# kdexd/virtex

Hardware: NVIDIA H100
Metric: image-caption pairs/sec bicaptioning R50-L1-H1024 (higher is better)
Workload: dtype bf16

## Files before the change

virtex_b200/csrc/gemm_tc.cu:

```cuda
#include <stdlib.h>
#include "ptx.cuh"
#include "vtx_common.cuh"
#include "../../include/virtex_b200.h"

#define KP_TAPS_W p.taps_w
#define KP_PAD p.pad
#define KP_NTAPS p.ntaps

namespace vtx {

constexpr int kBM = 128;
constexpr int kBK = 64;
constexpr int kMaxStages = 8;
constexpr int kABytes = kBM * kBK * 2;
constexpr int kSmemTotal = 232448;
constexpr int kCtrlBytes = 1024;
constexpr int kThreads = 384;
constexpr int kEpiThreads = 256;

struct FastDiv {
  uint32_t mul, shr;
};
__device__ __forceinline__ int fdiv(int x, const FastDiv& f) {
  return f.mul == 0u ? x : (int)(__umulhi((uint32_t)x, f.mul) >> f.shr);
// ... 675 lines not shown
        const int slabs = (min(p.bn, p.N - n_base) + 63) >> 6;
        for (int sl = 0; sl < slabs; ++sl) {
          if (p.mode & 1)
            tma_store_4d(&tmD, cbuf + sl * 16384, n_base + sl * 64, tw << p.lbw, th << p.lbh, tn << p.lbn);
          else
            tma_store_2d(&tmD, cbuf + sl * 16384, n_base + sl * 64, mt * kBM);
        }
        tma_store_commit();
      }
      if (bnr_on) {
        const uint32_t cp = smem_u32(cbuf) + (scg >> 3) * 16384 + bnr_r0 * 128;
        const int c8 = scg & 7;
        float mean[8], sc[8], sh[8];
        {
          const float4 m0 = __ldg(reinterpret_cast<const float4*>(p.bnr_bnp + bnr_col));
          const float4 m1 = __ldg(reinterpret_cast<const float4*>(p.bnr_bnp + bnr_col + 4));
          mean[0] = m0.x; mean[1] = m0.y; mean[2] = m0.z; mean[3] = m0.w;
          mean[4] = m1.x; mean[5] = m1.y; mean[6] = m1.z; mean[7] = m1.w;
          const float4 a0 = __ldg(reinterpret_cast<const float4*>(p.bnr_bnp + 2 * p.N + bnr_col));
          const float4 a1 = __ldg(reinterpret_cast<const float4*>(p.bnr_bnp + 2 * p.N + bnr_col + 4));
          const float4 b0 = __ldg(reinterpret_cast<const float4*>(p.bnr_bnp + 3 * p.N + bnr_col));
          const float4 b1 = __ldg(reinterpret_cast<const float4*>(p.bnr_bnp + 3 * p.N + bnr_col + 4));
          sc[0] = a0.x; sc[1] = a0.y; sc[2] = a0.z; sc[3] = a0.w; sc[4] = a1.x; sc[5] = a1.y; sc[6] = a1.z; sc[7] = a1.w;
          sh[0] = b0.x; sh[1] = b0.y; sh[2] = b0.z; sh[3] = b0.w; sh[4] = b1.x; sh[5] = b1.y; sh[6] = b1.z; sh[7] = b1.w;
        }
        for (int rb = 0; rb < st_rpt; rb += 4) {
          uint4 yv[4];
          uint32_t mbits;
          bnr_load(rb, yv, mbits);
#pragma unroll
          for (int r4 = 0; r4 < 4; ++r4) {
            const int r = rb + r4;
            const uint4 raw = lds128(cp + r * 128 + ((c8 ^ ((bnr_r0 + r) & 7)) << 4));
            float f[8], yy[8];
            unpack8(*reinterpret_cast<const bf16x8*>(&raw), f);
            unpack8(*reinterpret_cast<const bf16x8*>(&yv[r4]), yy);
#pragma unroll
            for (int i = 0; i < 8; ++i) {
              const bool on = p.bnr == 1 ? ((yy[i] * sc[i] + sh[i] > 0.f) && ((mbits >> (8 * r4)) & 0xffu) != 0u)
                                         : (((mbits >> (8 * r4 + i)) & 1u) != 0u);
              const float dz = on ? f[i] : 0.f;
              st_s[i] += dz;
              st_q[i] += dz * (yy[i] - mean[i]);
            }
          }
        }
      }
      if (!p.bnr && p.stats != nullptr && st_on) {
        const int r0 = srg * st_rpt;
        const uint32_t cp = smem_u32(cbuf) + (scg >> 3) * 16384 + r0 * 128;
        const int c8 = scg & 7;
        for (int rb = 0; rb < st_rpt; rb += 4) {
#pragma unroll
          for (int r4 = 0; r4 < 4; ++r4) {
            const int r = rb + r4;
            const uint4 raw = lds128(cp + r * 128 + ((c8 ^ ((r0 + r) & 7)) << 4));
            float f[8];
            unpack8(*reinterpret_cast<const bf16x8*>(&raw), f);
#pragma unroll
            for (int i = 0; i < 8; ++i) {
              st_s[i] += f[i];
              st_q[i] += f[i] * f[i];
            }
          }
        }
      }
    }
  }
  if (staged) {
    if (et == 0) tma_store_wait_read<0>();
    epi_bar(bar_id, epi_threads);
    if (p.stats != nullptr && st_nt >= 0) flush_stats(cstage0 + (PP ? (size_t)wg * p.cbytes : 0));
  }
}

typedef CUresult (*PFN_encodeTiled)(CUtensorMap*, CUtensorMapDataType, cuuint32_t, void*, const cuuint64_t*,
                                    const cuuint64_t*, const cuuint32_t*, const cuuint32_t*, CUtensorMapInterleave,
                                    CUtensorMapSwizzle, CUtensorMapL2promotion, CUtensorMapFloatOOBfill);

static PFN_encodeTiled get_encode() {
  static PFN_encodeTiled fn = nullptr;
  if (fn == nullptr) {
    void* p = nullptr;
    cudaDriverEntryPointQueryResult q;
    if (cudaGetDriverEntryPoint("cuTensorMapEncodeTiled", &p, cudaEnableDefault, &q) == cudaSuccess &&
        q == cudaDriverEntryPointSuccess)
      fn = reinterpret_cast<PFN_encodeTiled>(p);
  }
  return fn;
}

static int make_tmap(CUtensorMap* tm, const void* ptr, int rank, const uint64_t* dims, const uint64_t* strides_elems,
                     const uint32_t* box, const uint32_t* estr = nullptr) {
  PFN_encodeTiled enc = get_encode();
  if (!enc) return set_error(VTX_ECUDA, "cuTensorMapEncodeTiled entry point not available");
  cuuint64_t gdim[5];
  cuuint64_t gstr[5];
  cuuint32_t bx[5];
  cuuint32_t es[5];
  for (int i = 0; i < rank; ++i) {
    gdim[i] = dims[i];
    bx[i] = box[i];
    es[i] = estr ? estr[i] : 1;
  }
  for (int i = 0; i < rank - 1; ++i) gstr[i] = strides_elems[i] * 2;
  if ((reinterpret_cast<uintptr_t>(ptr) & 15) != 0) return set_error(VTX_EINVAL, "TMA base pointer not 16B aligned");
  for (int i = 0; i < rank - 1; ++i)
    if (gstr[i] % 16 != 0) return set_error(VTX_EINVAL, "TMA stride not a multiple of 16 bytes");
  CUresult r = enc(tm, CU_TENSOR_MAP_DATA_TYPE_BFLOAT16, (cuuint32_t)rank, const_cast<void*>(ptr), gdim, gstr, bx, es,
                   CU_TENSOR_MAP_INTERLEAVE_NONE, CU_TENSOR_MAP_SWIZZLE_128B, CU_TENSOR_MAP_L2_PROMOTION_L2_256B,
                   CU_TENSOR_MAP_FLOAT_OOB_FILL_NONE);
  if (r != CUDA_SUCCESS) return set_error(VTX_ECUDA, "cuTensorMapEncodeTiled failed (%d)", (int)r);
  return VTX_OK;
}

constexpr int kSchedSlots = 4096;
static int g_sched_dynamic = 0;
static struct SchedRing {
  unsigned int* ctr;
  unsigned int base[kSchedSlots];
  unsigned int next;
} g_sched[64];
static bool sched_is_dynamic() {
  static const char* env = getenv("VTX_GEMM_SCHEDULE");
  return env != nullptr ? (env[0] == 'd') : (g_sched_dynamic != 0);
}
static unsigned int* sched_slot(unsigned int fetches, unsigned int* base_out) {
  if (!sched_is_dynamic()) return nullptr;
  int dev = 0;
  cudaGetDevice(&dev);
  if (dev < 0 || dev >= 64) return nullptr;
  SchedRing& r = g_sched[dev];
  if (r.ctr == nullptr) {
    unsigned int* ptr = nullptr;
    if (cudaMalloc(&ptr, sizeof(unsigned int) * kSchedSlots) != cudaSuccess) return nullptr;
    cudaMemset(ptr, 0, sizeof(unsigned int) * kSchedSlots);
    cudaDeviceSynchronize();
    memset(r.base, 0, sizeof(r.base));
    r.next = 0;
    r.ctr = ptr;
  }
  const unsigned int slot = r.next++ % kSchedSlots;
  *base_out = r.base[slot];
  r.base[slot] += fetches;
  return r.ctr + slot;
}

static int ilog2(int x) {
  int l = 0;
  while ((1 << l) < x) ++l;
  return l;
}

static void choose_box(int H, int W, int positions, int* bw, int* bh, int* bn) {
  int best_w = 1, best_h = 1;
  double best_eff = -1;
  for (int w = 1; w <= positions; w <<= 1)
    for (int h = 1; w * h <= positions; h <<= 1) {
      if (w > 2 * W || h > 2 * H) continue;
      const int tw = (W + w - 1) / w, th = (H + h - 1) / h;
      const double eff = (double)(W * H) / ((double)tw * w * th * h);
      const double score = eff * 1000.0 + w * 0.01 + h * 0.0001;
      if (score > best_eff) { best_eff = score; best_w = w; best_h = h; }
    }
  *bw = best_w; *bh = best_h; *bn = positions / (best_w * best_h);
}

template <bool SS>
static cudaError_t launch_gemm(const cudaLaunchConfig_t& cfg, bool pingpong, int bn, const CUtensorMap& tmA,
                               const CUtensorMap& tmB, const CUtensorMap& tmD, const CUtensorMap& tmR,
                               const CUtensorMap& tmY, const GemmKParams& p) {
  if (pingpong && bn == 64) return cudaLaunchKernelEx(&cfg, gemm_wgmma_kernel<64, true, SS>, tmA, tmB, tmD, tmR, tmY, p);
  if (pingpong) return cudaLaunchKernelEx(&cfg, gemm_wgmma_kernel<128, true, SS>, tmA, tmB, tmD, tmR, tmY, p);
  if (bn == 64) return cudaLaunchKernelEx(&cfg, gemm_wgmma_kernel<64, false, SS>, tmA, tmB, tmD, tmR, tmY, p);
  if (bn == 128) return cudaLaunchKernelEx(&cfg, gemm_wgmma_kernel<128, false, SS>, tmA, tmB, tmD, tmR, tmY, p);
  if (bn == 192) return cudaLaunchKernelEx(&cfg, gemm_wgmma_kernel<192, false, SS>, tmA, tmB, tmD, tmR, tmY, p);
  return cudaLaunchKernelEx(&cfg, gemm_wgmma_kernel<256, false, SS>, tmA, tmB, tmD, tmR, tmY, p);
}

bool resid_dgrad_serves(const VtxGemm* g);
int resid_dgrad(const VtxGemm* g, cudaStream_t stream);

}

using namespace vtx;

extern "C" int vtx_gemm_set_dynamic_schedule(int on) {
  g_sched_dynamic = on ? 1 : 0;
  return VTX_OK;
}

extern "C" int vtx_gemm(const VtxGemm* g, void* stream_) {
  cudaStream_t stream = reinterpret_cast<cudaStream_t>(stream_);
  if (!g || !g->A || !g->B || !g->D) return set_error(VTX_EINVAL, "vtx_gemm: null pointer");
  if (g->M <= 0 || g->N <= 0 || g->K <= 0) return set_error(VTX_EINVAL, "vtx_gemm: empty problem");
  if (g->atomic && !g->out_f32) return set_error(VTX_EINVAL, "vtx_gemm: atomic accumulate needs fp32 output");
  if (g->split_k > 1 && !g->atomic) return set_error(VTX_EINVAL, "vtx_gemm: split_k > 1 needs atomic = 1");
  if (g->stats && (g->out_f32 || g->bias || g->residual || g->act || (g->alpha != 0.f && g->alpha != 1.f)))
    return set_error(VTX_EINVAL, "vtx_gemm: stats needs a plain bf16 output (no bias/residual/activation/alpha)");
  if (g->ldd % (g->out_f32 ? 4 : 8) != 0) return set_error(VTX_EINVAL, "vtx_gemm: ldd must keep rows 16B aligned");
  if (g->conv_mode < 0 || g->conv_mode > 6 || g->conv_mode == 3)
    return set_error(VTX_EINVAL, "vtx_gemm: conv_mode must be 0, 1, 2, 4, 5 or 6");
  VtxGemm g4;
  const bool trans_d = g->conv_mode == 4;
  if (trans_d) {
    if (g->conv_c != 64 || g->N != 64 || g->M != 9 * 64 || !g->out_f32 || !g->atomic)
      return set_error(VTX_EINVAL, "vtx_gemm: conv_mode 4 needs C = Cout = 64, M = 576, fp32 atomic output");
    g4 = *g;
    g4.conv_mode = 2;
    g4.M = g->N;
    g4.N = g->M;
    g4.split_k = vtx_num_sms() / 3;
    g4.conv_stride = 1;
    g4.conv_taps = 0;
    g = &g4;
  }
  const int split_k = g->split_k > 1 ? g->split_k : 1;

  GemmKParams p;
  memset(&p, 0, sizeof(p));
  p.M = g->M; p.N = g->N; p.K = g->K;
  p.a_mn = g->a_mn; p.b_mn = g->b_mn;
  p.mode = g->conv_mode;
  const bool stem = g->conv_mode == 5 || g->conv_mode == 6;
  p.taps_w = 3; p.pad = 1; p.ntaps = 9;
  if (stem) { p.mode = g->conv_mode == 5 ? 1 : 2; p.taps_w = 1; p.pad = 0; p.ntaps = 4; }
  const bool one_tap = !stem && g->conv_taps == 1;
  if (one_tap) { p.taps_w = 1; p.pad = 0; p.ntaps = 1; }
  const bool tap_grid = !stem && !one_tap && g->conv_taps_h > 0;
  if (tap_grid) {
    if (p.mode != 1 || g->conv_taps_w <= 0 || g->conv_taps_h > 3 || g->conv_taps_w > 3 || g->conv_pad < 0 || g->conv_pad > 1)
      return set_error(VTX_EINVAL, "vtx_gemm: bad explicit tap grid");
    p.taps_w = g->conv_taps_w; p.pad = g->conv_pad; p.ntaps = g->conv_taps_h * g->conv_taps_w;
  }
  const int cstride = (g->conv_stride == 2 && (p.mode == 1 || p.mode == 2) && !stem) ? 2 : 1;
  if (g->conv_stride != 0 && g->conv_stride != 1 && cstride != 2)
    return set_error(VTX_EINVAL, "vtx_gemm: conv_stride 2 is supported for conv_mode 1 / 2 only");
  if (g->conv_taps != 0 && g->conv_taps != 1 && g->conv_taps != 9) return set_error(VTX_EINVAL, "vtx_gemm: conv_taps must be 0, 1 or 9");
  p.cstride = cstride;
  const int ntaps = stem ? 4 : one_tap ? 1 : tap_grid ? p.ntaps : 9;
  if (p.mode == 1) { p.a_mn = 0; p.b_mn = 0; }
  if (p.mode == 2) { p.a_mn = 1; p.b_mn = 1; }
  int bn = g->tile_n;
  if (bn == 0) {
    const int gran = p.b_mn ? 64 : 16;
    if (g->N >= 256) bn = 256;
    else bn = ((g->N + gran - 1) / gran) * gran;
    if (bn == 256 && split_k == 1) {
      const long mt = (g->M + kBM - 1) / kBM;
      const long t256 = mt * ((g->N + 255) / 256);
      const int sms = vtx_num_sms();
      if (t256 < 100 || (t256 < sms && g->N % 256 != 0 && g->N <= 2048)) {
        bn = 128;
      } else if (t256 < 3L * sms && p.mode <= 1) {
        long best_cost = 0;
        int best_bn = 256;
        for (int cand = 256; cand >= 128; cand -= 64) {
          const long tiles = mt * ((g->N + cand - 1) / cand);
          const long cost = ((tiles + sms - 1) / sms) * (cand + 64);
          if (best_cost == 0 || cost < best_cost) { best_cost = cost; best_bn = cand; }
        }
        bn = best_bn;
      }
    }
  }
  if (bn < 16 || bn > 256 || bn % 16 != 0 || (p.b_mn && bn % 64 != 0))
    return set_error(VTX_EINVAL, "vtx_gemm: bad tile_n %d", bn);
  bn = bn <= 64 ? 64 : bn <= 128 ? 128 : bn <= 192 ? 192 : 256;
  const bool pingpong = bn <= 128 && !g->out_f32;
  p.bn = bn;
  p.n_tiles = (g->N + bn - 1) / bn;
  p.trans_d = trans_d ? 1 : 0;
  p.out_f32 = g->out_f32; p.atomic = g->atomic; p.act = g->act;
  p.alpha = g->alpha == 0.f ? 1.0f : g->alpha;
  p.D = g->D; p.ldd = g->ldd;
  p.bias = g->bias;
  p.bias_pairs = (g->bias != nullptr && g->N % 2 == 0 && (reinterpret_cast<uintptr_t>(g->bias) & 7) == 0) ? 1 : 0;
  p.residual = reinterpret_cast<const __nv_bfloat16*>(g->residual);
  p.ldr = g->ldr;
  p.res_mask = reinterpret_cast<const uint8_t*>(g->residual_mask);
  if (p.res_mask != nullptr && (g->residual == nullptr || g->N % 32 != 0 || g->conv_mode != 0 || g->out_f32 ||
                                (reinterpret_cast<uintptr_t>(g->residual_mask) & 3) != 0))
    return set_error(VTX_EINVAL, "vtx_gemm: residual_mask needs a residual, a plain bf16 GEMM and N %% 32 == 0");
  p.stats = g->stats;
  const bool bnr = g->bnr_y != nullptr;
  if (bnr) {
    if (!g->bnr_bnp || !g->bnr_sums || g->stats || g->out_f32 || g->bias || g->act || (g->alpha != 0.f && g->alpha != 1.f) ||
        g->N % 8 != 0 || g->bnr_ldy % 8 != 0 || (reinterpret_cast<uintptr_t>(g->bnr_y) & 15) != 0 ||
        (reinterpret_cast<uintptr_t>(g->bnr_bnp) & 15) != 0 || (g->bnr_mask != nullptr && g->conv_mode != 0) ||
        g->conv_mode == 2 || g->conv_mode >= 4 || split_k > 1)
      return set_error(VTX_EINVAL, "vtx_gemm: bnr needs a plain bf16 output (no stats/bias/activation/alpha/split-K), "
                                   "N %% 8 == 0, 16-byte aligned y / bnp; the bit-mask form needs conv_mode 0");
    if ((long long)g->M * (g->bnr_ldy > g->N ? g->bnr_ldy : g->N) >= (1ll << 31))
      return set_error(VTX_EUNSUPPORTED, "vtx_gemm: bnr needs M * ld(y) < 2^31");
    p.stats = g->bnr_sums;
    p.bnr_y = reinterpret_cast<const __nv_bfloat16*>(g->bnr_y);
    p.bnr_bnp = g->bnr_bnp;
    p.bnr_mask = g->bnr_mask;
    p.bnr_ldy = g->bnr_ldy;
    const char* pf = getenv("VTX_BNR_PREFETCH");
    p.bnr_prefetch = (pf != nullptr && pf[0] == '0') ? 0 : 1;
    p.bnr = g->bnr_mask == nullptr ? 1 : 2;
  }
  if (g->tile_n == 0 && resid_dgrad_serves(g)) return resid_dgrad(g, stream);
  const bool ss = g->col_scale != nullptr || g->col_shift != nullptr;
  if (ss) {
    if (!g->col_scale || !g->col_shift || g->out_f32 || (g->alpha != 0.f && g->alpha != 1.f) || g->bias || g->stats ||
        bnr || g->act < 0 || g->act > 1 || g->N % 2 != 0 || (reinterpret_cast<uintptr_t>(g->col_scale) & 7) != 0 ||
        (reinterpret_cast<uintptr_t>(g->col_shift) & 7) != 0 || g->residual_mask || g->conv_out_w > 0 ||
        (g->conv_mode != 0 && g->conv_mode != 1) ||
        (g->residual && (g->ldr % 8 != 0 || (reinterpret_cast<uintptr_t>(g->residual) & 15) != 0)))
      return set_error(VTX_EINVAL, "vtx_gemm: col_scale / col_shift need both vectors 8-byte aligned, a bf16 output, "
                                   "alpha 1, act 0 or 1, N %% 2 == 0, conv_mode 0 or 1 without an output view, no bias / "
                                   "stats / bnr / residual mask, and a 16-byte aligned residual with ldr %% 8 == 0");
    p.col_scale = g->col_scale;
    p.col_shift = g->col_shift;
  }

  CUtensorMap tmA, tmB;
  int rc;
  if (p.mode == 0) {
    p.m_tiles = (g->M + kBM - 1) / kBM;
    p.kb_total = (g->K + kBK - 1) / kBK;
    {
      uint64_t dims[2], str[1];
      uint32_t box[2];
      if (!p.a_mn) { dims[0] = g->K; dims[1] = g->M; box[0] = 64; box[1] = 128; }
      else { dims[0] = g->M; dims[1] = g->K; box[0] = 64; box[1] = 64; }
      str[0] = g->lda;
      if ((rc = make_tmap(&tmA, g->A, 2, dims, str, box)) != VTX_OK) return rc;
    }
    {
      uint64_t dims[2], str[1];
      uint32_t box[2];
      if (!p.b_mn) { dims[0] = g->K; dims[1] = g->N; box[0] = 64; box[1] = (uint32_t)bn; }
      else { dims[0] = g->N; dims[1] = g->K; box[0] = 64; box[1] = 64; }
      str[0] = g->ldb;
      if ((rc = make_tmap(&tmB, g->B, 2, dims, str, box)) != VTX_OK) return rc;
    }
  } else {
    const int C = g->conv_c, Hin = g->conv_h, Win = g->conv_w, NI = g->conv_n;
    const int H = (Hin - 1) / cstride + 1, W = (Win - 1) / cstride + 1;
    if (C <= 0 || C % 64 != 0) return set_error(VTX_EINVAL, "vtx_gemm: implicit conv needs channels %% 64 == 0");
    p.cH = H; p.cW = W; p.cN = NI; p.cpb = C / 64;
    const uint64_t xdims[4] = {(uint64_t)C, (uint64_t)Win, (uint64_t)(stem ? Hin + 3 : Hin), (uint64_t)NI};
    const uint64_t xstr[3] = {(uint64_t)(stem ? 16 : C), stem ? (uint64_t)(Win + 3) * 16 : (uint64_t)Win * C,
                              stem ? (uint64_t)(Hin + 3) * (Win + 3) * 16 : (uint64_t)Hin * Win * C};
    int bw, bh, bnn;
    choose_box(H, W, p.mode == 1 ? 128 : 64, &bw, &bh, &bnn);
    p.lbw = ilog2(bw); p.lbh = ilog2(bh); p.lbn = ilog2(bnn);
    p.tiles_w = (W + bw - 1) / bw;
    p.tiles_h = (H + bh - 1) / bh;
    const int tiles_n = (NI + bnn - 1) / bnn;
    if (p.mode == 1) {
      if (g->M != NI * H * W || g->K != ntaps * C) return set_error(VTX_EINVAL, "vtx_gemm: conv fprop shape mismatch");
      if (stem && g->stats && (W % bw != 0 || H % bh != 0))
        return set_error(VTX_EUNSUPPORTED, "vtx_gemm: conv_mode 5 with stats needs an output size tiled exactly by %dx%d", bw, bh);
      p.m_tiles = p.tiles_w * p.tiles_h * tiles_n;
      p.kb_total = ntaps * p.cpb;
      uint32_t box[4] = {64, (uint32_t)(bw * cstride), (uint32_t)(bh * cstride), (uint32_t)bnn};
      const uint32_t es[4] = {1, (uint32_t)cstride, (uint32_t)cstride, 1};
      if ((rc = make_tmap(&tmA, g->A, 4, xdims, xstr, box, cstride > 1 ? es : nullptr)) != VTX_OK) return rc;
      uint64_t bd[2] = {(uint64_t)g->K, (uint64_t)g->N};
      uint64_t bs[1] = {(uint64_t)g->ldb};
      uint32_t bb[2] = {64, (uint32_t)bn};
      if ((rc = make_tmap(&tmB, g->B, 2, bd, bs, bb)) != VTX_OK) return rc;
    } else {
      if (g->N != ntaps * C) return set_error(VTX_EINVAL, "vtx_gemm: conv wgrad shape mismatch");
      const int Cout = g->M;
      if (Cout % 64 != 0) return set_error(VTX_EINVAL, "vtx_gemm: conv wgrad needs Cout %% 64 == 0");
      p.m_tiles = (Cout + kBM - 1) / kBM;
      p.kb_total = p.tiles_w * p.tiles_h * tiles_n;
      uint64_t ad[4] = {(uint64_t)Cout, (uint64_t)W, (uint64_t)H, (uint64_t)NI};
      uint64_t as[3] = {(uint64_t)Cout, (uint64_t)W * Cout, (uint64_t)H * W * Cout};
      uint32_t box[4] = {64, (uint32_t)bw, (uint32_t)bh, (uint32_t)bnn};
      if ((rc = make_tmap(&tmA, g->A, 4, ad, as, box)) != VTX_OK) return rc;
      uint32_t xbox[4] = {64, (uint32_t)(bw * cstride), (uint32_t)(bh * cstride), (uint32_t)bnn};
      const uint32_t es[4] = {1, (uint32_t)cstride, (uint32_t)cstride, 1};
      if ((rc = make_tmap(&tmB, g->B, 4, xdims, xstr, xbox, cstride > 1 ? es : nullptr)) != VTX_OK) return rc;
    }
  }
  p.k_splits = split_k;
  if (p.k_splits > p.kb_total) p.k_splits = p.kb_total;
  p.kb_per_split = (p.kb_total + p.k_splits - 1) / p.k_splits;
  p.k_splits = (p.kb_total + p.kb_per_split - 1) / p.kb_per_split;

  p.stage_bytes = kABytes + bn * kBK * 2;
  p.cbytes = p.out_f32 ? 0 : ((bn + 63) / 64) * 16384;
  {
    const int kb_tile = p.kb_per_split;
    const int budget = kSmemTotal - 1024  - kCtrlBytes;
    int st = 0;
    p.nbuf = 1;
    if (pingpong) {
      p.nbuf = 2;
    } else if (p.cbytes) {
      const int st2 = (budget - 2 * p.cbytes) / p.stage_bytes;
      if (st2 >= 4 || (st2 >= 2 && st2 >= kb_tile)) { p.nbuf = 2; st = st2; }
    }
    if (st == 0) st = (budget - p.nbuf * p.cbytes) / p.stage_bytes;
    if (st > kMaxStages) st = kMaxStages;
    if (st < 2) return set_error(VTX_EUNSUPPORTED, "vtx_gemm: not enough shared memory for a 2-stage pipeline");
    p.stages = st;
  }
  CUtensorMap tmD, tmR, tmY;
  memset(&tmY, 0, sizeof(tmY));
  memset(&tmD, 0, sizeof(tmD));
  memset(&tmR, 0, sizeof(tmR));
  p.res_tma = (p.cbytes && g->residual != nullptr && g->ldr % 8 == 0 &&
               (reinterpret_cast<uintptr_t>(g->residual) & 15) == 0 && p.alpha == 1.0f && g->bias == nullptr &&
               (g->act == 0 || ss)) ? 1 : 0;
  if (p.cbytes) {
    if (p.mode & 1) {
      uint64_t dd[4] = {(uint64_t)g->N, (uint64_t)p.cW, (uint64_t)p.cH, (uint64_t)g->conv_n};
      uint64_t ds[3] = {(uint64_t)g->ldd, (uint64_t)p.cW * g->ldd, (uint64_t)p.cH * p.cW * g->ldd};
      if (g->conv_out_w > 0) {
        if (g->conv_out_h <= 0 || g->ldd_w % 8 || g->ldd_h % 8 || g->ldd_n % 8 || (g->residual != nullptr && !p.res_tma))
          return set_error(VTX_EINVAL, "vtx_gemm: bad output view");
        dd[1] = (uint64_t)g->conv_out_w; dd[2] = (uint64_t)g->conv_out_h;
        ds[0] = (uint64_t)g->ldd_w; ds[1] = (uint64_t)g->ldd_h; ds[2] = (uint64_t)g->ldd_n;
      }
      uint32_t db[4] = {64, 1u << p.lbw, 1u << p.lbh, 1u << p.lbn};
      if ((rc = make_tmap(&tmD, g->D, 4, dd, ds, db)) != VTX_OK) return rc;
      p.vW = (int)dd[1]; p.vH = (int)dd[2];
      if (bnr) {
        uint64_t ys[3] = {(uint64_t)g->bnr_ldy, (uint64_t)p.cW * g->bnr_ldy, (uint64_t)p.cH * p.cW * g->bnr_ldy};
        if (g->conv_out_w > 0) { ys[0] = ds[0]; ys[1] = ds[1]; ys[2] = ds[2]; }
        p.bnr_sw = (long long)ys[0]; p.bnr_sh = (long long)ys[1]; p.bnr_sn = (long long)ys[2];
        if ((rc = make_tmap(&tmY, g->bnr_y, 4, dd, ys, db)) != VTX_OK) return rc;
      }
      if (p.res_tma) {
        uint64_t rs[3] = {(uint64_t)g->ldr, (uint64_t)p.cW * g->ldr, (uint64_t)p.cH * p.cW * g->ldr};
        if (g->conv_out_w > 0) { rs[0] = ds[0]; rs[1] = ds[1]; rs[2] = ds[2]; }
        if ((rc = make_tmap(&tmR, g->residual, 4, dd, rs, db)) != VTX_OK) return rc;
      }
    } else {
      uint64_t dd[2] = {(uint64_t)g->N, (uint64_t)g->M};
      uint64_t ds[1] = {(uint64_t)g->ldd};
      uint32_t db[2] = {64, 128};
      if ((rc = make_tmap(&tmD, g->D, 2, dd, ds, db)) != VTX_OK) return rc;
      if (bnr) {
        uint64_t ys[1] = {(uint64_t)g->bnr_ldy};
        if ((rc = make_tmap(&tmY, g->bnr_y, 2, dd, ys, db)) != VTX_OK) return rc;
      }
      if (p.res_tma) {
        uint64_t rs[1] = {(uint64_t)g->ldr};
        if ((rc = make_tmap(&tmR, g->residual, 2, dd, rs, db)) != VTX_OK) return rc;
      }
    }
  }
  {
    static bool attr_set[64] = {false};
    int dev = 0;
    cudaGetDevice(&dev);
    if (dev < 0 || dev >= 64 || !attr_set[dev]) {
      cudaError_t e = cudaSuccess;
      const void* kernels[12] = {
// ... 47 lines not shown
```

Before: 6122.

## Add halo-tile implicit-GEMM kernels for 3x3 64-channel conv forward and wgrad

Adds specialized kernels for 3x3, stride-1, 64-channel convolutions. Each tile loads a padded spatial halo once via TMA and reuses it across all nine taps through offset wgmma descriptors, instead of gathering each tap separately. The forward path uses two ping-pong consumer warpgroups with plain, stats and BN-ReLU-backward epilogues. A separate wgrad kernel accumulates weight gradients from halo tiles and reduces them with vector red.add. Both use a dynamic atomic tile scheduler and are routed automatically when shapes qualify, at the cost of extra code paths and padding waste on partial tiles.

```diff
diff --git a/virtex_b200/csrc/gemm_halo.cu b/virtex_b200/csrc/gemm_halo.cu
--- /dev/null
+++ b/virtex_b200/csrc/gemm_halo.cu
@@ -0,0 +1,598 @@
+#include "ptx.cuh"
+#include "vtx_common.cuh"
+#include "../../include/virtex_b200.h"
+
+namespace vtx {
+
+namespace {
+
+constexpr int kHThreads = 288;
+constexpr int kHSmem = 232448;
+constexpr int kHCtrl = 1024;
+constexpr int kHMaxStages = 4;
+constexpr int kHTapBytes = 64 * 128;
+constexpr int kHOutBytes = 128 * 128;
+constexpr int kHRows = 128;
+
+enum { kEpiPlain = 0, kEpiStats = 1, kEpiBnr = 2 };
+
+struct HaloParams {
+  int H, W, NI;
+  int R, Wp;
+  int tiles_h, total;
+  int stages, halo_bytes;
+  uint32_t halo_tx;
+  int N;
+  float* sums;
+  const __nv_bfloat16* y;
+  long long ldy;
+  const float* bnp;
+  unsigned int* sched;
+  unsigned int sched_base;
+  float* dw;
+  int ldw;
+  int stage_bytes;
+};
+
+__device__ __forceinline__ void named_bar(int id, int threads) {
+  asm volatile("bar.sync %0, %1;" ::"r"(id), "r"(threads) : "memory");
+}
+__device__ __forceinline__ void sts32h(uint32_t a, uint32_t v) {
+  asm volatile("st.shared.b32 [%0], %1;" ::"r"(a), "r"(v) : "memory");
+}
+__device__ __forceinline__ uint4 ldg128_nc_h(const void* ptr) {
+  uint4 v;
+  asm volatile("ld.global.nc.L1::no_allocate.v4.b32 {%0, %1, %2, %3}, [%4];"
+               : "=r"(v.x), "=r"(v.y), "=r"(v.z), "=r"(v.w)
+               : "l"(ptr));
+  return v;
+}
+__device__ __forceinline__ uint32_t pack2(float lo, float hi) {
+  const __nv_bfloat162 h = __floats2bfloat162_rn(lo, hi);
+  return *reinterpret_cast<const uint32_t*>(&h);
+}
+__device__ __forceinline__ uint64_t halo_desc(uint32_t halo, uint32_t row, uint32_t kbytes) {
+  return make_wgmma_desc(halo + row * 128u + kbytes, 16, 1024);
+}
+
+template <int EPI>
+__global__ void __launch_bounds__(kHThreads, 1)
+halo_conv_kernel(const __grid_constant__ CUtensorMap tmX, const __grid_constant__ CUtensorMap tmW,
+                 const __grid_constant__ CUtensorMap tmD, const HaloParams p) {
+  VTX_PDL_TRIGGER();
+  extern __shared__ uint8_t smem_raw[];
+  uint8_t* base = reinterpret_cast<uint8_t*>((reinterpret_cast<uintptr_t>(smem_raw) + 1023) & ~uintptr_t(1023));
+  uint64_t* full_bar = reinterpret_cast<uint64_t*>(base);
+  uint64_t* empty_bar = full_bar + kHMaxStages;
+  uint64_t* order_bar = empty_bar + kHMaxStages;
+  uint64_t* w_bar = order_bar + 2;
+  volatile int* s_tile = reinterpret_cast<volatile int*>(base + 256);
+  uint8_t* sW = base + kHCtrl;
+  uint8_t* sOut = sW + 9 * kHTapBytes;
+  uint8_t* sHalo = sOut + 2 * kHOutBytes;
+
+  const int warp = __shfl_sync(0xffffffffu, (int)(threadIdx.x >> 5), 0);
+  const int lane = threadIdx.x & 31;
+
+  if (warp == 8 && lane == 0) {
+    tma_prefetch_desc(&tmX);
+    tma_prefetch_desc(&tmW);
+    tma_prefetch_desc(&tmD);
+    for (int i = 0; i < p.stages; ++i) {
+      mbar_init(&full_bar[i], 1);
+      mbar_init(&empty_bar[i], 1);
+    }
+    for (int i = 0; i < 2; ++i) mbar_init(&order_bar[i], 128);
+    mbar_init(w_bar, 1);
+    fence_mbar_init();
+  }
+  __syncthreads();
+  VTX_PDL_WAIT();
+
+  if (warp == 8) {
+    if (lane == 0) {
+      mbar_arrive_expect_tx(w_bar, 9u * kHTapBytes);
+      for (int tap = 0; tap < 9; ++tap) tma_load_2d(sW + tap * kHTapBytes, &tmW, w_bar, tap * 64, 0);
+      auto fetch = [&](int t_) -> int {
+        return p.sched != nullptr ? (int)(atomicAdd(p.sched, 1u) - p.sched_base) : t_;
+      };
+      int t = fetch((int)blockIdx.x);
+      for (int s = 0, ends = 0; ends < 2; ++s) {
+        const int stage = s % p.stages;
+        mbar_wait(&empty_bar[stage], ((uint32_t)(s / p.stages) & 1u) ^ 1u);
+        if (t < p.total) {
+          s_tile[stage] = t;
+          mbar_arrive_expect_tx(&full_bar[stage], p.halo_tx);
+          const int n = t / p.tiles_h, h0 = (t - n * p.tiles_h) * p.R;
+          tma_load_4d(sHalo + stage * p.halo_bytes, &tmX, &full_bar[stage], 0, -1, h0 - 1, n);
+          t = fetch(t + (int)gridDim.x);
+        } else {
+          s_tile[stage] = -1;
+          mbar_arrive(&full_bar[stage]);
+          ++ends;
+        }
+      }
+    }
+    return;
+  }
+
+  const int ct = threadIdx.x;
+  const int wg = ct >> 7;
+  const int wl = (ct >> 5) & 3;
+  const int et = ct & 127;
+  const int q = lane & 3;
+  const int sw = lane >> 2;
+  const int scg = et & 7, srg = et >> 3;
+  float st_s[8], st_q[8];
+#pragma unroll
+  for (int i = 0; i < 8; ++i) st_s[i] = st_q[i] = 0.f;
+  float mean[8], sc[8], sh[8];
+  if (EPI == kEpiBnr) {
+#pragma unroll
+    for (int i = 0; i < 8; ++i) {
+      mean[i] = __ldg(p.bnp + scg * 8 + i);
+      sc[i] = __ldg(p.bnp + 2 * p.N + scg * 8 + i);
+      sh[i] = __ldg(p.bnp + 3 * p.N + scg * 8 + i);
+    }
+  }
+
+  uint8_t* out = sOut + wg * kHOutBytes;
+  const uint32_t so = smem_u32(out);
+  const uint32_t sW0 = smem_u32(sW);
+  float acc[64];
+  mbar_wait(w_bar, 0);
+  for (int it = 0;; ++it) {
+    const int s = 2 * it + wg;
+    const int stage = s % p.stages;
+    const int round = s / p.stages;
+    if (round > 0) mbar_wait(&empty_bar[stage], (uint32_t)(round - 1) & 1u);
+    mbar_wait(&full_bar[stage], (uint32_t)round & 1u);
+    const int t = s_tile[stage];
+    if (t < 0) break;
+    if (wg == 1) mbar_wait(&order_bar[1], (uint32_t)it & 1u);
+    else if (it > 0) mbar_wait(&order_bar[0], (uint32_t)(it - 1) & 1u);
+
+    const uint32_t hb = smem_u32(sHalo + stage * p.halo_bytes);
+#pragma unroll
+    for (int i = 0; i < 64; ++i) fence_operand(acc[i]);
+    wgmma_fence();
+#pragma unroll
+    for (int tap = 0; tap < 9; ++tap) {
+      const uint32_t r0 = (uint32_t)((tap / 3) * p.Wp + tap % 3);
+#pragma unroll
+      for (int k = 0; k < 4; ++k) {
+        const uint64_t bd = make_wgmma_desc(sW0 + tap * kHTapBytes + k * 32, 16, 1024);
+        wgmma_n64<0, 0>(acc, halo_desc(hb, r0, k * 32), bd, (tap > 0 || k > 0) ? 1u : 0u);
+        wgmma_n64<0, 0>(acc + 32, halo_desc(hb, r0 + 64, k * 32), bd, (tap > 0 || k > 0) ? 1u : 0u);
+      }
+    }
+    wgmma_commit();
+    mbar_arrive(&order_bar[wg ^ 1]);
+    wgmma_wait<0>();
+#pragma unroll
+    for (int i = 0; i < 64; ++i) fence_operand(acc[i]);
+    if (et == 0) mbar_arrive(&empty_bar[stage]);
+
+    const int n = t / p.tiles_h, h0 = (t - n * p.tiles_h) * p.R;
+    const int rows_in = min(p.R, p.H - h0) * p.Wp;
+    if (et == 0) tma_store_wait_read<0>();
+    named_bar(1 + wg, 128);
+#pragma unroll
+    for (int hh = 0; hh < 4; ++hh) {
+      const int r = (hh >> 1) * 64 + wl * 16 + sw + 8 * (hh & 1);
+      const bool ok = r < rows_in && r % p.Wp < p.W;
+      const float* a = acc + (hh >> 1) * 32 + 2 * (hh & 1);
+      const uint32_t srow = so + r * 128 + q * 4;
+#pragma unroll
+      for (int j = 0; j < 8; ++j) sts32h(srow + ((j ^ sw) << 4), ok ? pack2(a[4 * j], a[4 * j + 1]) : 0u);
+    }
+    fence_proxy_async();
+    named_bar(1 + wg, 128);
+    if (et == 0) {
+      tma_store_4d(&tmD, out, 0, 0, h0, n);
+      tma_store_commit();
+    }
+
+    const uint32_t cp = so + srg * 8 * 128;
+    if (EPI == kEpiStats) {
+#pragma unroll
+      for (int r = 0; r < 8; ++r) {
+        const uint4 raw = lds128(cp + r * 128 + ((scg ^ r) << 4));
+        float f[8];
+        unpack8(*reinterpret_cast<const bf16x8*>(&raw), f);
+#pragma unroll
+        for (int i = 0; i < 8; ++i) {
+          st_s[i] += f[i];
+          st_q[i] += f[i] * f[i];
+        }
+      }
+    } else if (EPI == kEpiBnr) {
+      uint4 yv[8];
+      int r = srg * 8;
+      int rr = r / p.Wp, c = r - rr * p.Wp;
+      uint32_t okm = 0u;
+#pragma unroll
+      for (int i = 0; i < 8; ++i) {
+        const bool ok = r + i < rows_in && c < p.W;
+        const long long pos = ((long long)n * p.H + h0 + rr) * p.W + c;
+        yv[i] = ok ? ldg128_nc_h(p.y + pos * p.ldy + scg * 8) : make_uint4(0u, 0u, 0u, 0u);
+        okm |= (ok ? 1u : 0u) << i;
+        if (++c == p.Wp) { c = 0; ++rr; }
+      }
+#pragma unroll
+      for (int i = 0; i < 8; ++i) {
+        const uint4 raw = lds128(cp + i * 128 + ((scg ^ i) << 4));
+        float f[8], yy[8];
+        unpack8(*reinterpret_cast<const bf16x8*>(&raw), f);
+        unpack8(*reinterpret_cast<const bf16x8*>(&yv[i]), yy);
+#pragma unroll
+        for (int e = 0; e < 8; ++e) {
+          const bool on = (yy[e] * sc[e] + sh[e] > 0.f) && ((okm >> i) & 1u);
+          const float dz = on ? f[e] : 0.f;
+          st_s[e] += dz;
+          st_q[e] += dz * (yy[e] - mean[e]);
+        }
+      }
+    }
+  }
+  if (EPI != kEpiPlain) {
+    if (et == 0) tma_store_wait_read<0>();
+    named_bar(1 + wg, 128);
+    float* scr = reinterpret_cast<float*>(out);
+#pragma unroll
+    for (int i = 0; i < 8; i += 2)
+      *reinterpret_cast<float4*>(scr + (srg * 64 + scg * 8 + i) * 2) =
+          make_float4(st_s[i], st_q[i], st_s[i + 1], st_q[i + 1]);
+    named_bar(1 + wg, 128);
+    if (et < 64) {
+      float a = 0.f, b = 0.f;
+      for (int g = 0; g < 16; ++g) {
+        const float2 v = *reinterpret_cast<const float2*>(scr + (g * 64 + et) * 2);
+        a += v.x;
+        b += v.y;
+      }
+      if (EPI == kEpiBnr) b *= __ldg(p.bnp + p.N + et);
+      atomicAdd(p.sums + et, a);
+      atomicAdd(p.sums + p.N + et, b);
+    }
+  } else if (et == 0) {
+    tma_store_wait_read<0>();
+  }
+}
+
+typedef CUresult (*PFN_encode)(CUtensorMap*, CUtensorMapDataType, cuuint32_t, void*, const cuuint64_t*,
+                               const cuuint64_t*, const cuuint32_t*, const cuuint32_t*, CUtensorMapInterleave,
+                               CUtensorMapSwizzle, CUtensorMapL2promotion, CUtensorMapFloatOOBfill);
+
+int tmap_bf16(CUtensorMap* tm, const void* ptr, int rank, const uint64_t* dims, const uint64_t* strides,
+              const uint32_t* box) {
+  static PFN_encode enc = nullptr;
+  if (enc == nullptr) {
+    void* fp = nullptr;
+    cudaDriverEntryPointQueryResult qr;
+    if (cudaGetDriverEntryPoint("cuTensorMapEncodeTiled", &fp, cudaEnableDefault, &qr) != cudaSuccess ||
+        qr != cudaDriverEntryPointSuccess)
+      return set_error(VTX_ECUDA, "cuTensorMapEncodeTiled entry point not available");
+    enc = reinterpret_cast<PFN_encode>(fp);
+  }
+  cuuint64_t gd[4], gs[3];
+  cuuint32_t bx[4], es[4];
+  for (int i = 0; i < rank; ++i) {
+    gd[i] = dims[i];
+    bx[i] = box[i];
+    es[i] = 1;
+  }
+  for (int i = 0; i < rank - 1; ++i) gs[i] = strides[i] * 2;
+  const CUresult r = enc(tm, CU_TENSOR_MAP_DATA_TYPE_BFLOAT16, (cuuint32_t)rank, const_cast<void*>(ptr), gd, gs, bx, es,
+                         CU_TENSOR_MAP_INTERLEAVE_NONE, CU_TENSOR_MAP_SWIZZLE_128B, CU_TENSOR_MAP_L2_PROMOTION_L2_256B,
+                         CU_TENSOR_MAP_FLOAT_OOB_FILL_NONE);
+  if (r != CUDA_SUCCESS) return set_error(VTX_ECUDA, "cuTensorMapEncodeTiled failed (%d)", (int)r);
+  return VTX_OK;
+}
+
+bool al16h(const void* p) { return (reinterpret_cast<uintptr_t>(p) & 15) == 0; }
+
+struct HaloGeom {
+  int Wp, R, tiles_h, total, halo_bytes, stages;
+};
+HaloGeom halo_geom(const VtxGemm* g) {
+  HaloGeom h;
+  h.Wp = g->conv_w + 2;
+  h.R = kHRows / h.Wp;
+  h.tiles_h = h.R > 0 ? (g->conv_h + h.R - 1) / h.R : 0;
+  h.total = h.tiles_h * g->conv_n;
+  int rows = (h.R + 2) * h.Wp;
+  if (rows < 2 * h.Wp + 2 + kHRows) rows = 2 * h.Wp + 2 + kHRows;
+  h.halo_bytes = (rows * 128 + 1023) & ~1023;
+  const int fixed = 1024  + kHCtrl + 9 * kHTapBytes + 2 * kHOutBytes;
+  h.stages = (kHSmem - fixed) / h.halo_bytes;
+  if (h.stages > kHMaxStages) h.stages = kHMaxStages;
+  return h;
+}
+
+template <int EPI>
+cudaError_t launch_halo(const cudaLaunchConfig_t& cfg, const CUtensorMap& tmX, const CUtensorMap& tmW,
+                        const CUtensorMap& tmD, const HaloParams& p) {
+  cudaError_t e = cudaFuncSetAttribute(halo_conv_kernel<EPI>, cudaFuncAttributeMaxDynamicSharedMemorySize, kHSmem);
+  if (e != cudaSuccess) return e;
+  return cudaLaunchKernelEx(&cfg, halo_conv_kernel<EPI>, tmX, tmW, tmD, p);
+}
+
+constexpr int kWThreads = 416;
+constexpr int kWDyBytes = kHRows * 128;
+
+__global__ void __launch_bounds__(kWThreads, 1)
+halo_wgrad_kernel(const __grid_constant__ CUtensorMap tmX, const __grid_constant__ CUtensorMap tmY,
+                  const HaloParams p) {
+  VTX_PDL_TRIGGER();
+  extern __shared__ uint8_t smem_raw[];
+  uint8_t* base = reinterpret_cast<uint8_t*>((reinterpret_cast<uintptr_t>(smem_raw) + 1023) & ~uintptr_t(1023));
+  uint64_t* full_bar = reinterpret_cast<uint64_t*>(base);
+  uint64_t* empty_bar = full_bar + kHMaxStages;
+  volatile int* s_tile = reinterpret_cast<volatile int*>(base + 256);
+  uint8_t* sStage = base + kHCtrl;
+
+  const int warp = __shfl_sync(0xffffffffu, (int)(threadIdx.x >> 5), 0);
+  const int lane = threadIdx.x & 31;
+  const int xbox = (p.R + 2) * p.Wp * 128, ybox = p.R * p.Wp * 128;
+  if (warp == 12 && lane == 0) {
+    tma_prefetch_desc(&tmX);
+    tma_prefetch_desc(&tmY);
+    for (int i = 0; i < p.stages; ++i) {
+      mbar_init(&full_bar[i], 1);
+      mbar_init(&empty_bar[i], 3);
+    }
+    fence_mbar_init();
+  }
+  if (warp < 12) {
+    for (int s = 0; s < p.stages; ++s) {
+      const uint32_t st = smem_u32(sStage + s * p.stage_bytes);
+      for (int o = xbox + 16 * (int)threadIdx.x; o < p.halo_bytes; o += 16 * 384) sts128(st + o, 0u, 0u, 0u, 0u);
+      for (int o = ybox + 16 * (int)threadIdx.x; o < kWDyBytes; o += 16 * 384)
+        sts128(st + p.halo_bytes + o, 0u, 0u, 0u, 0u);
+    }
+    fence_proxy_async();
+  }
+  __syncthreads();
+  VTX_PDL_WAIT();
+
+  if (warp == 12) {
+    if (lane == 0) {
+      auto fetch = [&](int t_) -> int {
+        return p.sched != nullptr ? (int)(atomicAdd(p.sched, 1u) - p.sched_base) : t_;
+      };
+      int t = fetch((int)blockIdx.x);
+      for (int s = 0;; ++s) {
+        const int stage = s % p.stages;
+        mbar_wait(&empty_bar[stage], ((uint32_t)(s / p.stages) & 1u) ^ 1u);
+        if (t >= p.total) {
+          s_tile[stage] = -1;
+          mbar_arrive(&full_bar[stage]);
+          break;
+        }
+        s_tile[stage] = t;
+        mbar_arrive_expect_tx(&full_bar[stage], (uint32_t)(xbox + ybox));
+        const int n = t / p.tiles_h, h0 = (t - n * p.tiles_h) * p.R;
+        uint8_t* st = sStage + stage * p.stage_bytes;
+        tma_load_4d(st, &tmX, &full_bar[stage], 0, -1, h0 - 1, n);
+        tma_load_4d(st + p.halo_bytes, &tmY, &full_bar[stage], 0, 0, h0, n);
+        t = fetch(t + (int)gridDim.x);
+      }
+    }
+    return;
+  }
+
+  const int kh = threadIdx.x >> 7;
+  const int wl = (threadIdx.x >> 5) & 3;
+  float acc[96];
+#pragma unroll
+  for (int i = 0; i < 96; ++i) acc[i] = 0.f;
+  for (int s = 0;; ++s) {
+    const int stage = s % p.stages;
+    mbar_wait(&full_bar[stage], (uint32_t)(s / p.stages) & 1u);
+    if (s_tile[stage] < 0) break;
+    const uint32_t st = smem_u32(sStage + stage * p.stage_bytes);
+    const uint32_t r0 = (uint32_t)(kh * p.Wp);
+#pragma unroll
+    for (int i = 0; i < 96; ++i) fence_operand(acc[i]);
+    wgmma_fence();
+#pragma unroll
+    for (int k = 0; k < kHRows / 16; ++k) {
+      const uint64_t bd = make_wgmma_desc(st + p.halo_bytes + k * 2048, 8192, 1024);
+#pragma unroll
+      for (int j = 0; j < 3; ++j)
+        wgmma_n64<1, 1>(acc + 32 * j, make_wgmma_desc(st + (r0 + j + 16 * k) * 128, 8192, 1024), bd, 1u);
+    }
+    wgmma_commit();
+    wgmma_wait<0>();
+#pragma unroll
+    for (int i = 0; i < 96; ++i) fence_operand(acc[i]);
+    if ((threadIdx.x & 127) == 0) mbar_arrive(&empty_bar[stage]);
+  }
+  const int q = lane & 3;
+#pragma unroll
+  for (int j = 0; j < 3; ++j) {
+#pragma unroll
+    for (int hr = 0; hr < 2; ++hr) {
+      float* row = p.dw + (long long)((3 * kh + j) * 64 + wl * 16 + (lane >> 2) + 8 * hr) * p.ldw + 2 * q;
+#pragma unroll
+      for (int c = 0; c < 8; ++c) {
+        const float* a = acc + 32 * j + 4 * c + 2 * hr;
+        asm volatile("red.global.add.v2.f32 [%0], {%1, %2};" ::"l"(row + 8 * c), "f"(a[0]), "f"(a[1]) : "memory");
+      }
+    }
+  }
+}
+
+}
+
+bool halo_conv_serves(const VtxGemm* g) {
+  const bool bnr = g->bnr_y != nullptr;
+  if (g->conv_mode != 1 || g->conv_c != 64 || g->N != 64 || g->K != 576 || (g->conv_taps != 0 && g->conv_taps != 9) ||
+      g->conv_taps_h > 0 || (g->conv_stride != 0 && g->conv_stride != 1) || g->conv_out_w > 0)
+    return false;
+  if (g->out_f32 || g->atomic || g->split_k > 1 || g->act || g->bias || g->residual || g->residual_mask ||
+      (g->alpha != 0.f && g->alpha != 1.f) || g->col_scale || g->col_shift || (bnr && g->bnr_mask))
+    return false;
+  if (g->conv_w + 2 > kHRows || g->conv_h <= 0 || g->conv_n <= 0 ||
+      (long long)g->M != (long long)g->conv_n * g->conv_h * g->conv_w || halo_geom(g).stages < 2)
+    return false;
+  if (g->ldb % 8 || g->ldd % 8 || !al16h(g->A) || !al16h(g->B) || !al16h(g->D)) return false;
+  if (bnr && (!g->bnr_bnp || !g->bnr_sums || g->bnr_ldy % 8 || !al16h(g->bnr_y))) return false;
+  return true;
+}
+
+unsigned int halo_conv_fetches(const VtxGemm* g) {
+  const HaloGeom h = halo_geom(g);
+  const int sms = vtx_num_sms();
+  return (unsigned int)h.total + (unsigned int)(h.total < sms ? h.total : sms);
+}
+
+int halo_conv(const VtxGemm* g, cudaStream_t stream, unsigned int* sched, unsigned int sched_base) {
+  const HaloGeom h = halo_geom(g);
+  const int epi = g->bnr_y != nullptr ? kEpiBnr : g->stats != nullptr ? kEpiStats : kEpiPlain;
+  const uint64_t C = 64, W = (uint64_t)g->conv_w, H = (uint64_t)g->conv_h, NI = (uint64_t)g->conv_n;
+  CUtensorMap tmX, tmW, tmD;
+  int rc;
+  {
+    const uint64_t d[4] = {C, W, H, NI}, s[3] = {C, W * C, H * W * C};
+    const uint32_t b[4] = {64, (uint32_t)h.Wp, (uint32_t)(h.R + 2), 1};
+    if ((rc = tmap_bf16(&tmX, g->A, 4, d, s, b)) != VTX_OK) return rc;
+  }
+  {
+    const uint64_t d[2] = {(uint64_t)g->K, 64}, s[1] = {(uint64_t)g->ldb};
+    const uint32_t b[2] = {64, 64};
+    if ((rc = tmap_bf16(&tmW, g->B, 2, d, s, b)) != VTX_OK) return rc;
+  }
+  {
+    const uint64_t ld = (uint64_t)g->ldd;
+    const uint64_t d[4] = {64, W, H, NI}, s[3] = {ld, W * ld, H * W * ld};
+    const uint32_t b[4] = {64, (uint32_t)h.Wp, (uint32_t)h.R, 1};
+    if ((rc = tmap_bf16(&tmD, g->D, 4, d, s, b)) != VTX_OK) return rc;
+  }
+  HaloParams p;
+  memset(&p, 0, sizeof(p));
+  p.H = g->conv_h; p.W = g->conv_w; p.NI = g->conv_n;
+  p.R = h.R; p.Wp = h.Wp;
+  p.tiles_h = h.tiles_h; p.total = h.total;
+  p.stages = h.stages; p.halo_bytes = h.halo_bytes;
+  p.halo_tx = (uint32_t)((h.R + 2) * h.Wp * 128);
+  p.N = 64;
+  p.sums = epi == kEpiBnr ? g->bnr_sums : g->stats;
+  p.y = reinterpret_cast<const __nv_bfloat16*>(g->bnr_y);
+  p.ldy = g->bnr_ldy;
+  p.bnp = g->bnr_bnp;
+  p.sched = sched;
+  p.sched_base = sched_base;
+  const int sms = vtx_num_sms();
+  cudaLaunchConfig_t cfg;
+  memset(&cfg, 0, sizeof(cfg));
+  cfg.gridDim = dim3((unsigned)(h.total < sms ? h.total : sms));
+  cfg.blockDim = dim3(kHThreads);
+  cfg.dynamicSmemBytes = kHSmem;
+  cfg.stream = stream;
+  cudaLaunchAttribute attr[1];
+  attr[0].id = cudaLaunchAttributeProgrammaticStreamSerialization;
+  attr[0].val.programmaticStreamSerializationAllowed = 1;
+  cfg.attrs = attr;
+  cfg.numAttrs = 1;
+  const cudaError_t le = epi == kEpiBnr    ? launch_halo<kEpiBnr>(cfg, tmX, tmW, tmD, p)
+                         : epi == kEpiStats ? launch_halo<kEpiStats>(cfg, tmX, tmW, tmD, p)
+                                            : launch_halo<kEpiPlain>(cfg, tmX, tmW, tmD, p);
+  if (le != cudaSuccess) return set_error(VTX_ECUDA, "halo_conv_kernel launch: %s", cudaGetErrorString(le));
+  return VTX_OK;
+}
+
+void choose_box(int H, int W, int positions, int* bw, int* bh, int* bn);
+
+struct WgradPlan {
+  HaloGeom h;
+  int stage_bytes, stages, grid;
+};
+WgradPlan wgrad_plan(const VtxGemm* g) {
+  WgradPlan w;
+  w.h = halo_geom(g);
+  w.stage_bytes = w.h.halo_bytes + kWDyBytes;
+  w.stages = (kHSmem - 1024 - kHCtrl) / w.stage_bytes;
+  if (w.stages > kHMaxStages) w.stages = kHMaxStages;
+  w.grid = 0;
+  if (w.stages < 2 || w.h.total <= 0) return w;
+  int bw, bh, bnn;
+  choose_box(g->conv_h, g->conv_w, 64, &bw, &bh, &bnn);
+  const long kb_total = (long)((g->conv_w + bw - 1) / bw) * ((g->conv_h + bh - 1) / bh) * ((g->conv_n + bnn - 1) / bnn);
+  long splits = vtx_num_sms() / 3;
+  if (splits > kb_total) splits = kb_total;
+  if (splits < 1) splits = 1;
+  const long kbps = (kb_total + splits - 1) / splits;
+  const long depth = 4 * kbps + (kb_total + kbps - 1) / kbps;
+  const int T = w.h.total;
+  for (int grid = T < vtx_num_sms() ? T : vtx_num_sms(); grid >= 1; --grid) {
+    if (8L * ((T + grid - 1) / grid) + grid <= depth) {
+      w.grid = grid;
+      break;
+    }
+  }
+  return w;
+}
+
+bool halo_wgrad_serves(const VtxGemm* g) {
+  if (g->conv_mode != 4 || g->conv_c != 64 || g->N != 64 || g->M != 576 || !g->out_f32 || !g->atomic ||
+      (g->alpha != 0.f && g->alpha != 1.f) || (g->conv_taps != 0 && g->conv_taps != 9) ||
+      (g->conv_stride != 0 && g->conv_stride != 1) || g->bias || g->residual || g->stats || g->bnr_y || g->act)
+    return false;
+  if (g->conv_w + 2 > kHRows || g->conv_h <= 0 || g->conv_n <= 0 ||
+      (long long)g->K != (long long)g->conv_n * g->conv_h * g->conv_w)
+    return false;
+  if (g->ldd < 64 || g->ldd % 2 || (reinterpret_cast<uintptr_t>(g->D) & 7) || !al16h(g->A) || !al16h(g->B)) return false;
+  return wgrad_plan(g).grid > 0;
+}
+
+unsigned int halo_wgrad_fetches(const VtxGemm* g) {
+  const WgradPlan w = wgrad_plan(g);
+  return (unsigned int)w.h.total + (unsigned int)w.grid;
+}
+
+int halo_wgrad(const VtxGemm* g, cudaStream_t stream, unsigned int* sched, unsigned int sched_base) {
+  const WgradPlan w = wgrad_plan(g);
+  const HaloGeom& h = w.h;
+  const uint64_t C = 64, W = (uint64_t)g->conv_w, H = (uint64_t)g->conv_h, NI = (uint64_t)g->conv_n;
+  const uint64_t d[4] = {C, W, H, NI}, s[3] = {C, W * C, H * W * C};
+  CUtensorMap tmX, tmY;
+  int rc;
+  {
+    const uint32_t b[4] = {64, (uint32_t)h.Wp, (uint32_t)(h.R + 2), 1};
+    if ((rc = tmap_bf16(&tmX, g->B, 4, d, s, b)) != VTX_OK) return rc;
+  }
+  {
+    const uint32_t b[4] = {64, (uint32_t)h.Wp, (uint32_t)h.R, 1};
+    if ((rc = tmap_bf16(&tmY, g->A, 4, d, s, b)) != VTX_OK) return rc;
+  }
+  HaloParams p;
+  memset(&p, 0, sizeof(p));
+  p.H = g->conv_h; p.W = g->conv_w; p.NI = g->conv_n;
+  p.R = h.R; p.Wp = h.Wp;
+  p.tiles_h = h.tiles_h; p.total = h.total;
+  p.stages = w.stages; p.halo_bytes = h.halo_bytes; p.stage_bytes = w.stage_bytes;
+  p.N = 64;
+  p.dw = reinterpret_cast<float*>(g->D);
+  p.ldw = (int)g->ldd;
+  p.sched = sched;
+  p.sched_base = sched_base;
+  cudaLaunchConfig_t cfg;
+  memset(&cfg, 0, sizeof(cfg));
+  cfg.gridDim = dim3((unsigned)w.grid);
+  cfg.blockDim = dim3(kWThreads);
+  cfg.dynamicSmemBytes = kHSmem;
+  cfg.stream = stream;
+  cudaLaunchAttribute attr[1];
+  attr[0].id = cudaLaunchAttributeProgrammaticStreamSerialization;
+  attr[0].val.programmaticStreamSerializationAllowed = 1;
+  cfg.attrs = attr;
+  cfg.numAttrs = 1;
+  cudaError_t le = cudaFuncSetAttribute(halo_wgrad_kernel, cudaFuncAttributeMaxDynamicSharedMemorySize, kHSmem);
+  if (le == cudaSuccess) le = cudaLaunchKernelEx(&cfg, halo_wgrad_kernel, tmX, tmY, p);
+  if (le != cudaSuccess) return set_error(VTX_ECUDA, "halo_wgrad_kernel launch: %s", cudaGetErrorString(le));
+  return VTX_OK;
+}
+
+}
diff --git a/virtex_b200/csrc/gemm_tc.cu b/virtex_b200/csrc/gemm_tc.cu
--- a/virtex_b200/csrc/gemm_tc.cu
+++ b/virtex_b200/csrc/gemm_tc.cu
@@ -851,7 +851,7 @@
   return l;
 }
 
-static void choose_box(int H, int W, int positions, int* bw, int* bh, int* bn) {
+void choose_box(int H, int W, int positions, int* bw, int* bh, int* bn) {
   int best_w = 1, best_h = 1;
   double best_eff = -1;
   for (int w = 1; w <= positions; w <<= 1)
@@ -879,6 +879,12 @@
 
 bool resid_dgrad_serves(const VtxGemm* g);
 int resid_dgrad(const VtxGemm* g, cudaStream_t stream);
+bool halo_conv_serves(const VtxGemm* g);
+unsigned int halo_conv_fetches(const VtxGemm* g);
+int halo_conv(const VtxGemm* g, cudaStream_t stream, unsigned int* sched, unsigned int sched_base);
+bool halo_wgrad_serves(const VtxGemm* g);
+unsigned int halo_wgrad_fetches(const VtxGemm* g);
+int halo_wgrad(const VtxGemm* g, cudaStream_t stream, unsigned int* sched, unsigned int sched_base);
 
 }
 
@@ -900,6 +906,11 @@
   if (g->ldd % (g->out_f32 ? 4 : 8) != 0) return set_error(VTX_EINVAL, "vtx_gemm: ldd must keep rows 16B aligned");
   if (g->conv_mode < 0 || g->conv_mode > 6 || g->conv_mode == 3)
     return set_error(VTX_EINVAL, "vtx_gemm: conv_mode must be 0, 1, 2, 4, 5 or 6");
+  if (g->conv_mode == 4 && g->tile_n == 0 && halo_wgrad_serves(g)) {
+    unsigned int base = 0;
+    unsigned int* ctr = sched_slot(halo_wgrad_fetches(g), &base);
+    return halo_wgrad(g, stream, ctr, base);
+  }
   VtxGemm g4;
   const bool trans_d = g->conv_mode == 4;
   if (trans_d) {
@@ -1002,6 +1013,11 @@
     p.bnr = g->bnr_mask == nullptr ? 1 : 2;
   }
   if (g->tile_n == 0 && resid_dgrad_serves(g)) return resid_dgrad(g, stream);
+  if (g->tile_n == 0 && halo_conv_serves(g)) {
+    unsigned int base = 0;
+    unsigned int* ctr = sched_slot(halo_conv_fetches(g), &base);
+    return halo_conv(g, stream, ctr, base);
+  }
   const bool ss = g->col_scale != nullptr || g->col_shift != nullptr;
   if (ss) {
     if (!g->col_scale || !g->col_shift || g->out_f32 || (g->alpha != 0.f && g->alpha != 1.f) || g->bias || g->stats ||
```

Measured after the change: 6280, median of 6. 2.6% higher.
